# 3dlg-hcvc/tricolo

Measured on AMD Instinct MI355X. Metric: trimodal training samples/sec (32^3 voxel + 6-view), higher is better.
Workload: dtype f16 (f16 activation storage + f16 MFMA operands, fp32 accumulate; bf16x3 heads/GRU; within 1e-3 of the fp32 reference)

## Files before the change

### include/tricolo_hip.h

```cpp
#ifndef TRICOLO_HIP_H
#define TRICOLO_HIP_H
#include <stddef.h>
#include <stdint.h>

#ifdef __cplusplus
extern "C" {
#endif

#define TRI_FMT_F32 0
#define TRI_FMT_BF16 1
#define TRI_FMT_F16 2

int tri_version(void);
const char* tri_last_error(void);

typedef struct TriConvDesc {
    int B, ID, IH, IW, Cin;
    int OD, OH, OW, Cout;
    int KD, KH, KW, stride, pad_d, pad_h, pad_w;
} TriConvDesc;

int tri_conv_kpad(int ntaps, int cin_stored);
typedef struct TriPrepDesc {
    const float* w;
// ... 24 lines not shown

int tri_conv_num_mtiles(const TriConvDesc* d, int split3);
int tri_conv_num_records(const TriConvDesc* d, int split3, int row_list);
int tri_conv_kernel_family(const TriConvDesc* d, int transposed, int split3);
int tri_conv_wgrad_kernel_family(const TriConvDesc* d, int act_fmt);
size_t tri_conv_workspace(const TriConvDesc* d, int transposed);
int tri_conv_fwd(const TriConvDesc* d, const void* in, const void* w_hi, const void* w_lo, void* out, const uint8_t* row_mask,
                 const float* bias, int act, int accumulate, float* stats, int act_fmt, void* workspace, size_t workspace_bytes,
                 const int* row_pos , const int* row_count ,
                 void* stream);
int tri_conv_dgrad(const TriConvDesc* d, const void* dout, const void* wt_hi, const void* wt_lo, void* din, const uint8_t* row_mask,
                   int accumulate, int act_fmt, void* workspace, size_t workspace_bytes,
                   const int* row_pos ,
                   const int* row_count ,
                   void* stream);
typedef struct TriConvBnSums {
    const void* y;
    const float* relu_scale;
    const float* relu_shift;
    const void* relu_out;
    float* partial;
} TriConvBnSums;
int tri_conv_dgrad_bn_records(const TriConvDesc* d, int accumulate, int act_fmt);
int tri_conv_dgrad_bn(const TriConvDesc* d, const void* dout, const void* wt_hi, const void* wt_lo, void* din, int accumulate,
                      int act_fmt, void* workspace, size_t workspace_bytes, const int* row_pos, const TriConvBnSums* sums, void* stream);
size_t tri_conv_wgrad_workspace(const TriConvDesc* d);
size_t tri_conv_plan_bytes(const TriConvDesc* d);
int tri_conv_plan_build(const TriConvDesc* d, void* plan, void* stream);
int tri_conv_wgrad(const TriConvDesc* d, const void* in, const void* dout, const uint8_t* row_mask, const void* plan ,
                   void* workspace, size_t workspace_bytes, float* dw, long s_co, long s_tap, long s_ci, int cin_real, int split3,
                   int act_fmt, float out_scale ,
                   const int* row_pos, const int* row_count ,
                   void* stream);
#ifndef TRI_WGRAD_GROUP_MAX
#define TRI_WGRAD_GROUP_MAX 24
#endif
typedef struct TriWgradReduce {
    const float* slab;
    float* dw;
    long s_co, s_tap, s_ci;
    int splits, Cout, Kpad, ntaps, cin_stored, cin_real, zlanes, nblocks;
    float out_scale;
    int kw_real;
    int kw_shift;
} TriWgradReduce;
int tri_conv_wgrad_partial(const TriConvDesc* d, const void* in, const void* dout, const uint8_t* row_mask, const void* plan ,
// ... 154 lines not shown
```

### tricolo_amd/_C.py

```python
from __future__ import annotations

import ctypes as C
import os

import torch

_HERE = os.path.dirname(os.path.abspath(__file__))
LIB_PATH = os.path.join(_HERE, "libtricolo_hip.so")


class TriConvDesc(C.Structure):
    _fields_ = [(n, C.c_int) for n in ("B", "ID", "IH", "IW", "Cin", "OD", "OH", "OW", "Cout",
                                       "KD", "KH", "KW", "stride", "pad_d", "pad_h", "pad_w")]


class TriPrepDesc(C.Structure):
    _fields_ = [("w", C.c_void_p), ("hi", C.c_void_p), ("lo", C.c_void_p), ("s_row", C.c_long), ("s_tap", C.c_long),
                ("s_inner", C.c_long), ("rows", C.c_int), ("ntaps", C.c_int), ("inner", C.c_int), ("inner_pad", C.c_int),
                ("kpad", C.c_int), ("fmt", C.c_int), ("frag", C.c_int)]


class TriWgradReduce(C.Structure):
    _fields_ = [("slab", C.c_void_p), ("dw", C.c_void_p), ("s_co", C.c_long), ("s_tap", C.c_long), ("s_ci", C.c_long)] + \
               [(n, C.c_int) for n in ("splits", "Cout", "Kpad", "ntaps", "cin_stored", "cin_real", "zlanes", "nblocks")] + \
# ... 18 lines not shown

SIGNATURES = {
    "tri_version": (I, []),
    "tri_last_error": (C.c_char_p, []),
    "tri_conv_kpad": (I, [I, I]),
    "tri_weight_prep": (I, [P, L, L, L, I, I, I, I, P, P, I, I, P]),
    "tri_weight_prep_multi": (I, [P, I, P]),
    "tri_embedding_fwd": (I, [P, P, I, I, I, P, P]),
    "tri_embedding_bwd": (I, [P, P, I, I, I, I, I, P, P]),
    "tri_retrieval_topk": (I, [P, P, P, I, I, I, I, P, P, P, P]),
    "tri_linear_small_supported": (I, [I, I, I]),
    "tri_linear_small_fwd": (I, [P, P, P, P, I, I, I, I, I, P]),
    "tri_linear_small_dgrad": (I, [P, P, P, P, I, I, I, I, I, P]),
    "tri_linear_small_wgrad": (I, [P, P, P, P, P, I, I, I, I, I, P]),
    "tri_linear_small_bwd": (I, [P, P, P, P, P, P, P, I, I, I, I, I, P]),
    "tri_conv_num_mtiles": (I, [DP, I]),
    "tri_conv_num_records": (I, [DP, I, I]),
    "tri_conv_workspace": (Z, [DP, I]),
    "tri_conv_kernel_family": (I, [DP, I, I]),
    "tri_conv_wgrad_kernel_family": (I, [DP, I]),
    "tri_conv_fwd": (I, [DP, P, P, P, P, P, P, I, I, P, I, P, Z, P, P, P]),
    "tri_conv_dgrad": (I, [DP, P, P, P, P, P, I, I, P, Z, P, P, P]),
    "tri_conv_dgrad_bn_records": (I, [DP, I, I]),
    "tri_conv_dgrad_bn": (I, [DP, P, P, P, P, I, I, P, Z, P, C.POINTER(TriConvBnSums), P]),
    "tri_conv_wgrad_workspace": (Z, [DP]),
    "tri_conv_plan_bytes": (Z, [DP]),
    "tri_conv_plan_build": (I, [DP, P, P]),
    "tri_conv_wgrad": (I, [DP, P, P, P, P, P, Z, P, L, L, L, I, I, I, F, P, P, P]),
    "tri_conv_wgrad_partial": (I, [DP, P, P, P, P, P, Z, P, L, L, L, I, I, I, F, P, P, P, P]),
    "tri_wgrad_reduce_grouped": (I, [P, I, P]),
    "tri_wgrad_reduce_grouped_noted": (I, [P, I, P, P]),
    "tri_conv_stem_wgrad_bn": (I, [DP, P, P, P, P, P, P, P, P, P, P, Z, P, L, L, L, I, I, F, P, P]),
    "tri_conv_wgrad_group_info": (I, [DP, I, P, P, P]),
    "tri_conv_wgrad_partial_group": (I, [P, I, I, P, P]),
    "tri_bn_finalize": (I, [P, I, I, P, I, P, P, P, P, P, F, F, P, P, P, P, P]),
    "tri_bn_eval_coeffs": (I, [I, P, P, P, P, F, P, P, P, P, P]),
    "tri_bn_act": (I, [P, P, P, P, P, P, P, L, I, I, I, P]),
    "tri_relu_bwd": (I, [P, P, P, L, I, P]),
    "tri_bn_bwd_num_blocks": (I, [L]),
    "tri_bn_bwd_reduce": (I, [P, P, L, I, P, P, P, P, P, I, P]),
    "tri_bn_bwd_finalize": (I, [P, I, I, P, I, P, P, P, P, P, P, P, P, F, P]),
    "tri_bn_bwd_small": (I, [P, P, L, I, P, I, P, P, P, P, P, P, P, P, I, P, P, P, F, I, P]),
    "tri_bn_bwd_apply": (I, [P, P, P, P, P, P, P, L, I, P, P, P, P, I, I, P]),
    "tri_bn_bwd_pair_reduce": (I, [P, P, P, P, L, I, P, P, I, P]),
    "tri_bn_bwd_pair_finalize": (I, [P, P, I, I, I, P, P, P, P, P, P, P, P, F, P]),
    "tri_bn_bwd_pair_apply": (I, [P, P, P, P, P, P, P, P, P, L, I, I, P]),
# ... 130 lines not shown
```

### tricolo_amd/csrc/conv_igemm.hip

```cpp
#include "common.h"
#include <stdlib.h>
#include <map>
#include <mutex>
#include "../../include/tricolo_hip.h"
#include "conv_vox.h"

struct ConvArgs {
    const void* in;
    const void* w_hi;
    const void* w_lo;
    void* out;
    const uint8_t* row_mask;
    const int* row_pos;
    const int* row_count;
    const float* bias;
    float* stats;
    float* slab;
    int B, ID, IH, IW, Cin;
    int OD, OH, OW, Cout;
    int KD, KH, KW, stride, pd, ph, pw;
    int transposed, act, accumulate;
    int Kpad, M, ntaps, cin_shift, ksplit, steps_per_split;
    unsigned in_bytes;
    int nunits;
    int h_tr, h_rows, h_slab_bytes, h_nr, h_mtiles;
    int h_dbuf;
    int h_abl;
    int h_xcg, h_touch;
    int h_swz;
#ifdef HALO_STAMPS
    long long* h_dbg;
#endif
    FastDiv dOW, dOH, dOD, dCin, dP, dH2;
};

template <int N>
__device__ __forceinline__ float row_ror(float v) {
    return __builtin_bit_cast(float, __builtin_amdgcn_update_dpp(0, __builtin_bit_cast(int, v), 0x120 + N, 0xf, 0xf, false));
}

template <typename AT, int BN, int TM, int TN, int WAVES_M, int WM, int WN>
__device__ __forceinline__ void conv_epilogue(const ConvArgs& p, f32x4 (&acc)[TM][TN], int m0, int n0, int mtile, int wm, int wn, int fr,
                                              int fq, int t, int split, int any_active, float* red, int Meff) {
    if (p.ksplit > 1) {
        if (!any_active) return;
        float* slab = p.slab + (size_t)split * p.M * p.Cout;
#pragma unroll
        for (int a = 0; a < TM; ++a) {
            int m = m0 + wm * WM + a * 16 + fr;
            if (m < Meff)
#pragma unroll
                for (int b = 0; b < TN; ++b) {
                    int n = n0 + wn * WN + b * 16 + fq * 4;
                    *(f32x4*)(slab + (size_t)m * p.Cout + n) = acc[a][b];
                }
        }
// ... 544 lines not shown
        stats[((size_t)rec * 2 + 1) * Cout + ntile * BN + t] = q_;
    }
}

__device__ __forceinline__ v4i lds_read16(unsigned addr) {
    v4i r;
    asm volatile("ds_read_b128 %0, %1" : "=v"(r) : "v"(addr));
    return r;
}
template <int OFF>
__device__ __forceinline__ v4i lds_read16_off(unsigned addr) {
    v4i r;
    asm volatile("ds_read_b128 %0, %1 offset:%2" : "=v"(r) : "v"(addr), "n"(OFF));
    return r;
}
template <int N>
__device__ __forceinline__ void frag_wait(v4i (&a)[2], v4i (&b)[4]) {
    asm volatile("s_waitcnt lgkmcnt(%6)" : "+v"(a[0]), "+v"(a[1]), "+v"(b[0]), "+v"(b[1]), "+v"(b[2]), "+v"(b[3]) : "n"(N));
}
template <int N>
__device__ __forceinline__ void frag_wait(v4i (&a)[3], v4i (&b)[4]) {
    asm volatile("s_waitcnt lgkmcnt(%7)" : "+v"(a[0]), "+v"(a[1]), "+v"(a[2]), "+v"(b[0]), "+v"(b[1]), "+v"(b[2]), "+v"(b[3]) : "n"(N));
}
#ifdef HALO_STAMPS
#define HSTAMP(id) do { if (wave == 0 && n_stamp < 255) { const long long c_ = __builtin_readcyclecounter(); if (lane == 0) stl[n_stamp] = ((long long)(id) << 48) | (c_ & 0xFFFFFFFFFFFFll); ++n_stamp; } } while (0)
#else
#define HSTAMP(id) do { } while (0)
#endif
template <int TM, bool WGREC, typename AT>
__global__ __launch_bounds__(256, WGREC ? 3 : 1) void conv_halo2d_kernel(const ConvArgs p) {
    typedef Mma<typename OpOf<AT>::E> MM;
    typedef typename MM::v8 v8;
    constexpr int BN = 64, TN = 4, WM = 16 * TM, W_BYTES = BN * 128, NR = HALO_NR;
    extern __shared__ __attribute__((aligned(16))) char smem[];
    const int slab_bytes = p.h_slab_bytes;
    char* const ring = smem + slab_bytes;
    float* const red = (float*)(ring + NR * W_BYTES);

    const int t = threadIdx.x, lane = t & 63, wave = t >> 6;
    const int fr = lane & 15, fq = lane >> 4;
#ifdef HALO_STAMPS
    int n_stamp = 0;
    long long* const stl = (long long*)(smem + p.h_slab_bytes + HALO_NR * 8192 + 2048);
#endif
    HSTAMP(1);
    const int H = p.IH, W = p.IW, P = W + 2, TR = p.h_tr, NH = p.B * H;
    const int NT = p.Cout / BN, nchunks = p.Cin >> 6;
    const int items = p.h_mtiles * NT, G = gridDim.x;
    const int S = slab_bytes >> 12;
    const int zero_pix = p.h_rows * P;
    const v4i in_rsrc = make_rsrc_words(p.in, p.in_bytes);
    const v4i w_rsrc = make_rsrc_words(p.w_hi, (unsigned)((size_t)p.Cout * p.Kpad * 2));
    const unsigned lds_slab = lds_addr(smem) + wave * 1024, lds_ring = lds_addr(ring) + wave * 1024;
// ... 76 lines not shown
        }
    };

    int item = blockIdx.x;
    if (item >= items) return;
    HSTAMP(2);
    {
        issue_slab((item / NT) * TR, 0);
#pragma unroll
        for (int d = 0; d < NR - 1; ++d) issue_w();
    }
    int c_slot = 0;
    f32x4 cs[TN], cq[TN];
#pragma unroll
    for (int b = 0; b < TN; ++b) { cs[b] = (f32x4){0.f, 0.f, 0.f, 0.f}; cq[b] = cs[b]; }
    for (; item < items; item += G) {
        const int mtile = item / NT, ntile = item - mtile * NT;
        if (!WGREC) {
#pragma unroll
            for (int b = 0; b < TN; ++b) { cs[b] = (f32x4){0.f, 0.f, 0.f, 0.f}; cq[b] = cs[b]; }
        }
        const int g0 = mtile * TR;
        const int npos = min(TR, NH - g0) * W;
        int pix0[TM], tmul[TM];
#pragma unroll
        for (int a = 0; a < TM; ++a) {
            const bool ok = wave * WM + a * 16 + fr < npos;
            pix0[a] = ok ? pixc[a] : zero_pix;
            tmul[a] = ok ? 1 : 0;
        }
        f32x4 acc[TM][TN];
#pragma unroll
        for (int a = 0; a < TM; ++a)
#pragma unroll
            for (int b = 0; b < TN; ++b) acc[a][b] = (f32x4){0.f, 0.f, 0.f, 0.f};

        for (int chunk = 0; chunk < nchunks; ++chunk) {
            if (chunk > 0) {
                __builtin_amdgcn_s_barrier();
                asm volatile("" ::: "memory");
                issue_slab(g0, chunk);
            }
            HSTAMP(3);
            asm volatile("s_waitcnt vmcnt(0)" ::: "memory");
            HSTAMP(4);
            int shift = p.transposed ? (P + 1) : -(P + 1), kx = 0;
            int gshift = p.transposed ? (p.h_swz + 1) : -(p.h_swz + 1);
#pragma unroll 1
            for (int tap = 0; tap < 9; ++tap) {
                --w_ahead;
                if (tap > 0 && !(p.h_abl & 64)) {
                    if (w_ahead == NR - 2) wait_vmcnt_c<2 * (NR - 2)>();
                    else wait_vmcnt(2 * w_ahead);
                }
                HSTAMP(5);
                __builtin_amdgcn_s_barrier();
                asm volatile("" ::: "memory");
                HSTAMP(6);
// ... 14 lines not shown
                        for (int a = 0; a < TM; ++a) ar[kk][a] = lds_read16(aaddr[a] ^ (kk << 6));
#pragma unroll
                        for (int b = 0; b < TN; ++b) br[kk][b] = lds_read16_off<0>(wb + boff[kk] + b * 2048);
                    }
                    frag_wait<TM + TN>(ar[0], br[0]);
#pragma unroll
                    for (int b = 0; b < TN; ++b)
#pragma unroll
                        for (int a = 0; a < TM; ++a) acc[a][b] = MM::mma(__builtin_bit_cast(v8, br[0][b]), __builtin_bit_cast(v8, ar[0][a]), acc[a][b]);
                    frag_wait<0>(ar[1], br[1]);
#pragma unroll
                    for (int b = 0; b < TN; ++b)
#pragma unroll
                        for (int a = 0; a < TM; ++a) acc[a][b] = MM::mma(__builtin_bit_cast(v8, br[1][b]), __builtin_bit_cast(v8, ar[1][a]), acc[a][b]);
                }
                HSTAMP(8);
                if (++c_slot == NR) c_slot = 0;
                const int step = (++kx == 3) ? (kx = 0, P - 2) : 1;
                const int gstep = kx == 0 ? p.h_swz - 2 : 1;
                shift += p.transposed ? -step : step;
                gshift += p.transposed ? -gstep : gstep;
            }
        }
        __builtin_amdgcn_s_barrier();
        asm volatile("" ::: "memory");
        if (item + G < items) issue_slab(((item + G) / NT) * TR, 0);

        HSTAMP(9);
        if (!(p.h_abl & 4)) {
            AT* const out = (AT*)p.out + ((size_t)g0 * W) * p.Cout + ntile * BN;
#pragma unroll
            for (int a = 0; a < TM; ++a) {
                const int m = wave * WM + a * 16 + fr;
                if (m < npos) {
#pragma unroll
                    for (int b = 0; b < TN; ++b) {
                        AT* o = out + (size_t)m * p.Cout + b * 16 + fq * 4;
                        f32x4 v = acc[a][b];
                        if (p.accumulate) { float4 e = Act<AT>::ld4(o); v[0] += e.x; v[1] += e.y; v[2] += e.z; v[3] += e.w; }
                        Act<AT>::st4(o, make_float4(v[0], v[1], v[2], v[3]));
                        if (p.stats) {
                            v[0] = Act<AT>::rnd(v[0]); v[1] = Act<AT>::rnd(v[1]); v[2] = Act<AT>::rnd(v[2]); v[3] = Act<AT>::rnd(v[3]);
                            cs[b] += v;
                            cq[b] += v * v;
                        }
                    }
                }
            }
            HSTAMP(10);
            if (!WGREC && p.stats && !(p.h_abl & 16)) halo_store_stats<TN, BN>(cs, cq, red, p.stats, p.Cout, mtile, ntile, wave, fr, fq, t, true);
        }
        HSTAMP(11);
    }
#ifdef HALO_STAMPS
    if (wave == 0) {
        asm volatile("s_waitcnt lgkmcnt(0)" ::: "memory");
        for (int i = lane; i < 255; i += 64) p.h_dbg[(size_t)blockIdx.x * 256 + i] = i < n_stamp ? stl[i] : 0;
        if (lane == 0) p.h_dbg[(size_t)blockIdx.x * 256 + 255] = n_stamp;
    }
#endif
    if (WGREC && p.stats && !(p.h_abl & 16)) halo_store_stats<TN, BN>(cs, cq, red, p.stats, p.Cout, blockIdx.x / NT, blockIdx.x % NT, wave, fr, fq, t, false);
}


// ... 1180 lines not shown
                for (int tap = 0; tap < 9; ++tap)
                    for (int kk = 0; kk < 2; ++kk)
                        for (int g = 0; g < 4; ++g) {
                            int cnt[16] = {0}, mx = 0;
                            for (int l = 0; l < 16; ++l) {
                                const int lane = grp[g][l], fr = lane & 15, fq = lane >> 4;
                                const int pa = wave * 16 * TM + a * 16 + fr, j = pa / W, x = pa - j * W, i = whole ? j / H : 0;
                                const int row = j + 1 + 2 * i + tap / 3 - 1, col = x + 1 + tap % 3 - 1;
                                const int slot = (((row * P + col) & 1) << 3) | (((fq + 4 * kk) ^ (col + c1 * row)) & 7);
                                if (++cnt[slot] > mx) mx = cnt[slot];
                            }
                            cyc += mx;
                        }
        if (best < 0 || cyc < best) { best = cyc; best_c = c1; }
    }
    std::lock_guard<std::mutex> lk(mu);
    memo[key] = best_c;
    return best_c;
}

#ifdef HALO_STAMPS
static long long* g_halo_dbg = nullptr;
#endif
template <int TM, typename AT>
static int launch_halo(ConvArgs& a, const ConvPlan& pl, hipStream_t stream) {
    a.h_tr = pl.h_tr; a.h_rows = pl.h_rows; a.h_slab_bytes = pl.h_slab_bytes; a.h_nr = pl.h_nr; a.h_mtiles = pl.h_mtiles;
    a.h_dbuf = pl.h_dbuf;
    a.h_abl = tri_probe_ablation();
    a.dP = make_fastdiv(a.IW + 2); a.dH2 = make_fastdiv(a.IH + 2);
    a.h_swz = halo_swizzle(a.IW, a.IH, pl.halo);
#ifdef HALO_STAMPS
    a.h_dbg = g_halo_dbg;
    const size_t smem = (size_t)pl.h_slab_bytes + (size_t)HALO_NR * 8192 + 2048 + 2048;
#else
    const size_t smem = (size_t)pl.h_slab_bytes + (size_t)HALO_NR * 8192 + 2048;
#endif
    a.h_xcg = 0; a.h_touch = 0;
    if (pl.h_v5) {
        static int xcg_on = -1, touch_on = -1;
        if (xcg_on < 0) { const char* e = getenv("TRICOLO_HALO_XCG"); xcg_on = e ? atoi(e) : -1; if (xcg_on < 0) xcg_on = 99; }
        if (touch_on < 0) { const char* e = getenv("TRICOLO_HALO_TOUCH"); touch_on = (e && e[0] == '0') ? 0 : 1; }
        const int NT = a.Cout / 64, G = pl.h_grid;
        if (xcg_on && G == pl.h_mtiles * NT && G % 8 == 0 && a.Cin != 64) {
            const double wb = (double)a.Cout * a.Kpad * 2, ib = (double)a.M * a.Cin * 2;
            double best = 0;
            for (int cg = 1; cg <= NT; ++cg) {
                if (NT % cg || 8 % (NT / cg) || (G / 8) % cg) continue;
                if (xcg_on != 99 && cg != xcg_on) continue;
// ... 14 lines not shown
#ifdef HALO_NTL_EXPERIMENT
        { static int f = -1; if (f < 0) f = 0;
          const int items = pl.h_mtiles * (a.Cout / 64), per_wg = (items + pl.h_grid - 1) / pl.h_grid;
          if (f && a.Cin != 64 && per_wg > 1) ntl = per_wg == 2 ? 2 : 4; }
#endif
#define TRI_ROWS_LAUNCH(DRIP_, ACC_, NTL_, ...)                                                                                     \
        do {                                                                                                                        \
            static size_t attr5 = 0;                                                                                                \
            if (smem5 > attr5) {                                                                                                    \
                hipFuncSetAttribute((const void*)conv_halo_rows_kernel<AT, DRIP_, ACC_, NTL_, ##__VA_ARGS__>, hipFuncAttributeMaxDynamicSharedMemorySize, \
                                    (int)smem5);                                                                                    \
                attr5 = smem5;                                                                                                      \
            }                                                                                                                       \
            conv_halo_rows_kernel<AT, DRIP_, ACC_, NTL_, ##__VA_ARGS__><<<pl.h_grid, 256, smem5, stream>>>(a);                       \
        } while (0)
#define TRI_ROWS_MODE(NTL_)                                                                                                         \
        do {                                                                                                                        \
            if (a.accumulate) TRI_ROWS_LAUNCH(false, true, NTL_);                                                                   \
            else if (drip) TRI_ROWS_LAUNCH(true, false, NTL_);                                                                      \
            else TRI_ROWS_LAUNCH(false, false, NTL_);                                                                               \
        } while (0)
        static int prod = -1;
        if (prod < 0) { const char* e = getenv("TRICOLO_HALO_PROD"); prod = (e && e[0] == '0') ? 0 : 1; }
        if (prod && pl.halo == 2 && ntl == 0) {
#define TRI_ROWS_LAUNCH_P(DRIP_, ACC_)                                                                                              \
        do {                                                                                                                        \
            static size_t attrp = 0;                                                                                                \
            if (smem5 > attrp) {                                                                                                    \
                hipFuncSetAttribute((const void*)conv_halo_rows_kernel<AT, DRIP_, ACC_, 0, 2, true>, hipFuncAttributeMaxDynamicSharedMemorySize, \
                                    (int)smem5);                                                                                    \
                attrp = smem5;                                                                                                      \
            }                                                                                                                       \
            conv_halo_rows_kernel<AT, DRIP_, ACC_, 0, 2, true><<<pl.h_grid, 512, smem5, stream>>>(a);                                \
        } while (0)
            if (a.accumulate) TRI_ROWS_LAUNCH_P(false, true);
            else if (drip) TRI_ROWS_LAUNCH_P(true, false);
            else TRI_ROWS_LAUNCH_P(false, false);
#undef TRI_ROWS_LAUNCH_P
            return tri_check_launch("tri_conv(halo rows, producer waves)");
        }
        if (pl.halo == 3) {
            if (a.accumulate) TRI_ROWS_LAUNCH(false, true, 0, 3);
            else TRI_ROWS_LAUNCH(false, false, 0, 3);
        }
        else if (ntl == 0) TRI_ROWS_MODE(0);
        else if (ntl == 1) TRI_ROWS_MODE(1);
#ifdef HALO_NTL_EXPERIMENT
        else if (ntl == 2) TRI_ROWS_MODE(2);
        else TRI_ROWS_MODE(4);
#endif
#undef TRI_ROWS_MODE
#undef TRI_ROWS_LAUNCH
        return tri_check_launch("tri_conv(halo rows)");
    }
    static size_t attr = 0;
    if (smem > attr) {
        hipFuncSetAttribute((const void*)conv_halo2d_kernel<TM, false, AT>, hipFuncAttributeMaxDynamicSharedMemorySize, (int)smem);
        hipFuncSetAttribute((const void*)conv_halo2d_kernel<TM, true, AT>, hipFuncAttributeMaxDynamicSharedMemorySize, (int)smem);
        attr = smem;
    }
    if (pl.h_wgrec && a.stats) conv_halo2d_kernel<TM, true, AT><<<pl.h_grid, 256, smem, stream>>>(a);
    else conv_halo2d_kernel<TM, false, AT><<<pl.h_grid, 256, smem, stream>>>(a);
    return tri_check_launch("tri_conv(halo)");
}

template <typename AT>
static int launch_stem(ConvArgs& a, hipStream_t stream) {
    StemGeom sg;
    a.h_abl = tri_probe_ablation();
    if (!stem_geometry(a.B, a.IH, a.IW, a.Cin, a.OH, a.OW, a.Cout, a.KD, a.KH, a.KW, a.stride, a.pd, a.ph, a.pw, &sg)) {
        tri_set_error("conv(stem): geometry changed between plan and launch"); return TRI_ERR_ARG;
    }
    const size_t smem = (size_t)2 * sg.slab_rows * sg.row_bytes + 4 * 64 * 2 * sizeof(float);
#define TRI_STEM(KH_)                                                                                                     \
    case KH_: {                                                                                                           \
        static bool attr = false;                                                                                         \
        if (!attr) {                                                                                                      \
            hipFuncSetAttribute((const void*)conv_stem_kernel<KH_, 2, AT>, hipFuncAttributeMaxDynamicSharedMemorySize, 80 * 1024); \
            hipFuncSetAttribute((const void*)conv_stem_kernel<KH_, 4, AT>, hipFuncAttributeMaxDynamicSharedMemorySize, 80 * 1024); \
            attr = true;                                                                                                  \
        }                                                                                                                 \
        if (sg.npt == 4) conv_stem_kernel<KH_, 4, AT><<<sg.grid, 256, smem, stream>>>(a, sg);                             \
// ... 94 lines not shown
            return tri_internal_c64_launch(cg, a.B, a.IH, a.in, a.w_hi, a.out, bs ? bs->partial : a.stats, a.transposed, a.accumulate, act_fmt, bs, stream);
        }
        if (a.stats) {
            tri_set_error("conv: this layer runs conv_c64_kernel (tri_conv_kernel_family == 9): statistics only without row mask / bias / activation");
            return TRI_ERR_ARG;
        }
        a.row_pos = a.row_count ? a.row_pos : nullptr;
    }
    if (pl.s2g) {
        if (a.transposed || a.row_mask || a.row_count || a.bias || a.act != 0 || a.accumulate) {
            tri_set_error("conv: this layer runs conv_s2g_kernel (tri_conv_kernel_family == 15): forward only, no row mask / list, bias, activation "
                          "or accumulate");
            return TRI_ERR_ARG;
        }
        TriS2gGeom g2;
        tri_internal_s2g_geometry(a.B, a.ID, a.IH, a.IW, a.Cin, a.OD, a.OH, a.OW, a.Cout, a.KD, a.KH, a.KW, a.stride, a.pd, a.ph, a.pw, &g2);
        return tri_internal_s2g_launch(g2, a.B, a.IH, a.IW, a.Cin, a.Cout, a.Kpad, a.in, a.w_hi, a.out, a.stats, act_fmt, stream);
    }
    if (pl.s2d && a.transposed && !bs && !a.row_mask && !a.row_count && !a.bias && a.act == 0 && !a.stats) {
        TriC64Geom sg;
        tri_internal_s2d_geometry(a.B, a.ID, a.IH, a.IW, a.Cin, a.OD, a.OH, a.OW, a.Cout, a.KD, a.KH, a.KW, a.stride, a.pd, a.ph, a.pw, &sg);
        return tri_internal_s2d_launch(sg, a.B, a.IH, a.in, a.w_hi, a.out, a.accumulate, act_fmt, stream);
    }
    if (bs) {
        tri_set_error("conv: this layer's data-gradient kernel takes no BatchNorm-backward sums (tri_conv_dgrad_bn_records == 0)");
        return TRI_ERR_UNSUPPORTED;
    }
    if (pl.stem && !a.transposed && !a.row_mask && !a.row_count && !a.bias && a.act == 0 && !a.accumulate) {
        a.row_pos = nullptr;
        return act_fmt == TRI_FMT_F16 ? launch_stem<f16_t>(a, stream) : launch_stem<bf16_t>(a, stream);
    }
    if (pl.halo && !a.row_mask && !a.row_count && !a.bias && a.act == 0) {
        a.row_pos = nullptr;
        return act_fmt == TRI_FMT_F16 ? launch_halo<2, f16_t>(a, pl, stream) : launch_halo<2, bf16_t>(a, pl, stream);
    }
    if (pl.pw && pl.pw_tr == (a.transposed ? 1 : 0) && !a.row_mask && !a.row_count && !a.bias && a.act == 0 && !a.accumulate) {
        TriPwGeom pg;
        tri_internal_pw_geometry(a.B, a.ID, a.IH, a.IW, a.Cin, a.OD, a.OH, a.OW, a.Cout, a.KD, a.KH, a.KW, a.stride, a.pd, a.ph, a.pw, &pg);
        return tri_internal_pw_launch(pg, a.B, a.in, a.w_hi, a.Cin, a.Cout, a.Kpad, a.out, a.stats, a.transposed ? 1 : 0, act_fmt, stream);
    }
    if (pl.dma) return act_fmt == TRI_FMT_F16 ? launch_dma_any<f16_t>(a, pl.bn, stream) : launch_dma_any<bf16_t>(a, pl.bn, stream);
#define TRI_CONV(BN_)                                                                                     \
    (act_fmt == TRI_FMT_F16 ? launch_conv<BN_, 1, f16_t>(a, stream)                                       \
     : act_fmt == TRI_FMT_BF16 ? launch_conv<BN_, 1, bf16_t>(a, stream)                                   \
     : (split ? launch_conv<BN_, 2, float>(a, stream) : launch_conv<BN_, 1, float>(a, stream)))
    if (a.Cout % 128 == 0 && pl.bn != 64) return TRI_CONV(128);
    if (a.Cout % 64 == 0) return TRI_CONV(64);
    return TRI_CONV(32);
#undef TRI_CONV
}

extern "C" int tri_conv_kpad(int ntaps, int cin_stored) { return (ntaps * cin_stored + 31) / 32 * 32; }

extern "C" int tri_conv_num_records(const TriConvDesc* d, int split3, int row_list) {
    long M = (long)d->B * d->OD * d->OH * d->OW;
    ConvPlan pl = conv_make_plan(d->B, d->ID, d->IH, d->IW, d->Cin, d->OD, d->OH, d->OW, d->Cout, d->KD, d->KH, d->KW, d->stride, d->pad_d,
                                 d->pad_h, d->pad_w, split3, row_list);
// ... 66 lines not shown
extern "C" int tri_conv_dgrad(const TriConvDesc* d, const void* dout, const void* wt_hi, const void* wt_lo, void* din,
                              const uint8_t* row_mask, int accumulate, int act_fmt, void* workspace, size_t workspace_bytes,
                              const int* row_pos, const int* row_count, void* stream) {
    ConvArgs a{};
    a.in = dout; a.w_hi = wt_hi; a.w_lo = wt_lo; a.out = din;
    a.row_mask = row_mask; a.bias = nullptr; a.stats = nullptr; a.row_pos = row_pos; a.row_count = row_count;
    a.B = d->B; a.ID = d->OD; a.IH = d->OH; a.IW = d->OW; a.Cin = d->Cout;
    a.OD = d->ID; a.OH = d->IH; a.OW = d->IW; a.Cout = d->Cin;
    a.KD = d->KD; a.KH = d->KH; a.KW = d->KW; a.stride = d->stride; a.pd = d->pad_d; a.ph = d->pad_h; a.pw = d->pad_w;
    a.transposed = 1; a.act = 0; a.accumulate = accumulate;
    a.ntaps = d->KD * d->KH * d->KW;
    a.M = d->B * d->ID * d->IH * d->IW;
    return conv_dispatch(a, act_fmt, workspace, workspace_bytes, (hipStream_t)stream);
}

extern "C" int tri_conv_dgrad_bn_records(const TriConvDesc* d, int accumulate, int act_fmt) {
    (void)accumulate;
    if (act_fmt != TRI_FMT_BF16 && act_fmt != TRI_FMT_F16) return 0;
    ConvPlan pl = conv_make_plan(d->B, d->OD, d->OH, d->OW, d->Cout, d->ID, d->IH, d->IW, d->Cin, d->KD, d->KH, d->KW, d->stride, d->pad_d,
                                 d->pad_h, d->pad_w, 2, 0);
    if (pl.c64 && d->IW <= 32) return pl.c64_grid;
    return 0;
}
extern "C" int tri_conv_dgrad_bn(const TriConvDesc* d, const void* dout, const void* wt_hi, const void* wt_lo, void* din, int accumulate,
                                 int act_fmt, void* workspace, size_t workspace_bytes, const int* row_pos, const TriConvBnSums* sums,
                                 void* stream) {
    if (!sums || !sums->y || !sums->partial || (!sums->relu_scale != !sums->relu_shift) || (sums->relu_scale && sums->relu_out)) {
        tri_set_error("tri_conv_dgrad_bn: sums needs y, partial and at most one of (relu_scale + relu_shift) / relu_out");
        return TRI_ERR_ARG;
    }
    if (tri_conv_dgrad_bn_records(d, accumulate, act_fmt) == 0) {
        tri_set_error("tri_conv_dgrad_bn: no fused form for this layer (tri_conv_dgrad_bn_records == 0)");
        return TRI_ERR_UNSUPPORTED;
    }
    ConvArgs a{};
    a.in = dout; a.w_hi = wt_hi; a.w_lo = wt_lo; a.out = din;
    a.row_pos = row_pos;
    a.B = d->B; a.ID = d->OD; a.IH = d->OH; a.IW = d->OW; a.Cin = d->Cout;
    a.OD = d->ID; a.OH = d->IH; a.OW = d->IW; a.Cout = d->Cin;
    a.KD = d->KD; a.KH = d->KH; a.KW = d->KW; a.stride = d->stride; a.pd = d->pad_d; a.ph = d->pad_h; a.pw = d->pad_w;
    a.transposed = 1; a.act = 0; a.accumulate = accumulate;
    a.ntaps = d->KD * d->KH * d->KW;
    a.M = d->B * d->ID * d->IH * d->IW;
    return conv_dispatch(a, act_fmt, workspace, workspace_bytes, (hipStream_t)stream, sums);
}
```

### tricolo_amd/model/module/img_encoder/mv_cnn.py

```python
from __future__ import annotations

import os

import torch
import torch.nn as nn

from .... import ops
from ....layers import SideStream, TriModule, linear_bwd, linear_fwd, require_gpu


_DS_FWD = int(os.environ.get("TRICOLO_DS_FWD", "2"))
_DS_BWD = int(os.environ.get("TRICOLO_DS_BWD", "2"))
_PREP_DGRAD_LATE = os.environ.get("TRICOLO_PREP_DGRAD_LATE", "1") != "0"
_BN_PAIR = True
_STEM_BESIDE_WGRAD = os.environ.get("TRICOLO_STEM_BESIDE_WGRAD", "1") != "0"
_PREP_ISSUE = int(os.environ.get("TRICOLO_PREP_ISSUE", "1"))


class _BasicBlockParams(nn.Module):
    def __init__(self, inplanes, planes, stride):
        super().__init__()
        self.conv1 = nn.Conv2d(inplanes, planes, 3, stride, 1, bias=False)
        self.bn1 = nn.BatchNorm2d(planes)
        self.relu = nn.ReLU(inplace=True)
# ... 279 lines not shown
            g = dout
            fine = ops.TIMELINE is not None and ops.TIMELINE.get("fine")
            tag = f"image.bwd.c{y2.shape[-1]}.b{bi}"
            if fine:
                ops.stamp(tag + ".bn2")
            mode = _DS_BWD if (blk.downsample is not None and batch is not None) else 0
            ev = None
            if mode == 2:
                ev = torch.cuda.Event()
                ev.record()

            def shortcut_bwd():
                with torch.cuda.stream(self._side_ds.fork(g, yd, event=ev)):
                    if dyd_pair is not None:
                        return dyd_pair, ops.conv_dgrad(dyd_pair, gd, self._packed[(id(blk.downsample[0]), True)])
                    dyd_, gr[blk.downsample[1].weight], gr[blk.downsample[1].bias] = ops.bn_bwd(
                        yd, g, cod, blk.downsample[1].weight, count_host=gd.M, inplace=False, out_scale=ugs)
                    if batch is None:
                        gr[blk.downsample[0].weight] = ops.conv_wgrad(x, dyd_, gd, blk.downsample[0].weight, prec, out_scale=ugs)
                    return dyd_, ops.conv_dgrad(dyd_, gd, self._packed[(id(blk.downsample[0]), True)])
            if blk.downsample is not None and not mode:
                dyd, dx = shortcut_bwd()
            wgrad_async(a1, dy2, g2, blk.conv2.weight)
            da1, sums1 = ops.conv_dgrad(dy2, g2, self._packed[(id(blk.conv2), True)], bn_sums=(y1, co1, None))
            if mode:
                dyd, dx = shortcut_bwd()
            if fine:
                ops.stamp(tag + ".dgrad2")
            dy1, gr[blk.bn1.weight], gr[blk.bn1.bias] = ops.bn_bwd(y1, da1, co1, blk.bn1.weight, count_host=g1.M, relu=True, out_scale=ugs,
                                                                   partial=sums1)
            if fine:
                ops.stamp(tag + ".bn1")
            wgrad_async(x, dy1, g1, blk.conv1.weight)
            if blk.downsample is not None:
                if batch is None:
                    self._side_ds.join(dx, gr[blk.downsample[0].weight], gr[blk.downsample[1].weight], gr[blk.downsample[1].bias])
                else:
                    self._side_ds.join(dx, dyd, gr[blk.downsample[1].weight], gr[blk.downsample[1].bias])
                    gr[blk.downsample[0].weight] = ops.conv_wgrad(x, dyd, gd, blk.downsample[0].weight, prec, out_scale=ugs, batch=batch)
            else:
                dx = g
            if bi > 0:
                prev = saved_blocks[bi - 1]
                dx, dout_sums = ops.conv_dgrad(dy1, g1, self._packed[(id(blk.conv1), True)], out=dx, accumulate=True,
                                               bn_sums=(prev[5], None, prev[11]))
            else:
                dx, dout_sums = ops.conv_dgrad(dy1, g1, self._packed[(id(blk.conv1), True)], out=dx, accumulate=True), None
# ... 134 lines not shown
```

### tricolo_amd/ops.py

```python
from __future__ import annotations

import math
import os

import torch

from . import _C
from ._C import check, lib, make_desc, ptr, stream

_PRECISIONS = ("bf16", "bf16x3", "f16")
_FMT = {torch.float32: 0, torch.bfloat16: 1, torch.float16: 2}
F16_GRAD_SCALE = float(os.environ.get("TRICOLO_F16_GRAD_SCALE", "4096"))
if not (F16_GRAD_SCALE >= 1.0 and math.frexp(F16_GRAD_SCALE)[0] == 0.5):
    raise ValueError(f"TRICOLO_F16_GRAD_SCALE={F16_GRAD_SCALE!r}: must be a power of two >= 1 (the kernels divide it out exactly)")
_default_precision = os.environ.get("TRICOLO_PRECISION", "bf16x3")


def set_default_precision(p: str):
    global _default_precision
    if p not in _PRECISIONS:
        raise ValueError(f"precision must be one of {_PRECISIONS}")
    _default_precision = p


# ... 198 lines not shown
        return t

    def brick(self, transposed: bool, mode: int) -> bool:
        return (self.kernel_family[(transposed, mode)] & 255) in (6, 7, 13, 14)

    def packed_frag(self, transposed: bool, precision: str, storage=None) -> int:
        storage = storage or act_dtype(precision)
        mode = 1 if precision == "bf16x3" else (2 if storage != torch.float32 else 0)
        return 1 if (self.kernel_family[(transposed, mode)] & 255) in _FRAG_FAMILIES else 0

    def check_packed(self, packed, transposed: bool, x):
        need = 1 if (self.kernel_family[(transposed, _conv_mode(x, packed[1]))] & 255) in _FRAG_FAMILIES else 0
        if getattr(packed[0], "tri_frag", 0) != need:
            raise RuntimeError("conv: the packed operand was ordered for another plan (row-major vs fragment-major): pack it with "
                               "pack_weight(..., storage=<dtype of the activations>)")

    def voxg_spu(self, transposed: bool, mode: int) -> int:
        code = self.kernel_family[(transposed, mode)]
        return (code >> 24) & 127 if (code & 255) == 13 else 0

    def splitk(self, transposed: bool, mode: int) -> bool:
        return bool(self.kernel_family[(transposed, mode)] >> 16 & 1)

    def dgrad_bn_records(self, accumulate: bool, fmt: int) -> int:
        c = self.__dict__.setdefault("_dgrad_bn", {})
        k = (bool(accumulate), fmt)
        if k not in c:
            c[k] = int(lib().tri_conv_dgrad_bn_records(_C.C.byref(self.desc), 1 if accumulate else 0, fmt))
        return c[k]

    def wgrad_group(self, fmt: int):
        c = self.__dict__.setdefault("_wgrad_group", {})
        if fmt not in c:
            fam, tiles, steps = _C.C.c_int(), _C.C.c_int(), _C.C.c_int()
            check(lib().tri_conv_wgrad_group_info(_C.C.byref(self.desc), fmt, _C.C.byref(fam), _C.C.byref(tiles), _C.C.byref(steps)),
                  "tri_conv_wgrad_group_info")
            c[fmt] = (fam.value, tiles.value, steps.value)
        return c[fmt]

    def plan(self, device):
        pl = self._plans.get(device)
        if pl is None:
            pl = torch.empty((lib().tri_conv_plan_bytes(_C.C.byref(self.desc)),), dtype=torch.uint8, device=device)
            check(lib().tri_conv_plan_build(_C.C.byref(self.desc), ptr(pl), stream()), "tri_conv_plan_build")
            self._plans[device] = pl
        return pl

    @property
    def flops(self):
        return 2 * self.M * self.ntaps * self.cin * self.cout

# ... 63 lines not shown
    g.check_packed(packed, False, x)
    OD, OH, OW = g.out_grid
    if out is None:
        out = torch.empty((g.B, OD, OH, OW, g.cout), dtype=x.dtype, device=x.device)
    assert out.dtype == x.dtype
    nrec = (g.num_records_rows if rows else g.num_mtiles)[_conv_mode(x, lo)]
    stats = torch.empty((nrec, 2, g.cout), dtype=torch.float32, device=x.device) if want_stats else None
    ws = _workspace(g.fwd_ws, x.device) if g.fwd_ws else None
    check(_timed(_igemm_symbol(g, False, lo is not None, x), _flops(g, rows, row_mask),
                 lambda: lib().tri_conv_fwd(_C.C.byref(g.desc), ptr(_act(x)), ptr(hi), ptr(lo), ptr(out), ptr(row_mask), ptr(bias),
                                            act, 1 if accumulate else 0, ptr(stats), _abf(x), ptr(ws),
                                            ws.numel() if ws is not None else 0, ptr(rows[0]) if rows else None,
                                            ptr(rows[1]) if rows else None, stream())), "tri_conv_fwd")
    return (out, stats) if want_stats else out


_ROW_ORDER = True


_DGRAD_BN_MODE = os.environ.get("TRICOLO_DGRAD_BN", "2")
_DGRAD_BN = _DGRAD_BN_MODE != "0"


def conv_dgrad(dout, g: ConvGeom, packed_t, row_mask=None, out=None, accumulate=False, rows=None, bn_sums=None):
    hi, lo = packed_t
    g.check_packed(packed_t, True, dout)
    ID, IH, IW = g.in_grid
    if out is None:
        out = torch.empty((g.B, ID, IH, IW, g.cin_stored), dtype=dout.dtype, device=dout.device)
    assert out.dtype == dout.dtype
    ws = _workspace(g.dgrad_ws, dout.device) if g.dgrad_ws else None
    rowpos = g.dgrad_row_order(dout.device) if (row_mask is None and rows is None and _ROW_ORDER) else None
    if rows is not None:
        rowpos = rows[0]
    if bn_sums is not None:
        y, co, relu_out = bn_sums
        nrec = g.dgrad_bn_records(accumulate, _abf(dout)) if (_DGRAD_BN and not (accumulate and _DGRAD_BN_MODE == "2") and row_mask is None and rows is None and lo is None
                                                               and (relu_out is not None) == bool(accumulate)
                                                               and (co is not None) != (relu_out is not None)) else 0
        if nrec == 0:
            return conv_dgrad(dout, g, packed_t, row_mask=row_mask, out=out, accumulate=accumulate, rows=rows), None
        assert y.dtype == out.dtype and y.numel() == out.numel()
        partial = torch.empty((nrec, 2, g.cin_stored), dtype=torch.float32, device=dout.device)
        sums = _C.TriConvBnSums(ptr(y), ptr(co.scale) if co is not None else None, ptr(co.shift) if co is not None else None,
                                ptr(relu_out), ptr(partial))
        check(_timed(_igemm_symbol(g, True, False, dout), g.flops,
                     lambda: lib().tri_conv_dgrad_bn(_C.C.byref(g.desc), ptr(_act(dout)), ptr(hi), None, ptr(out), 1 if accumulate else 0,
                                                     _abf(dout), ptr(ws), ws.numel() if ws is not None else 0, ptr(rowpos),
                                                     _C.C.byref(sums), stream())), "tri_conv_dgrad_bn")
        return out, partial
    check(_timed(_igemm_symbol(g, True, lo is not None, dout), _flops(g, rows, row_mask),
                 lambda: lib().tri_conv_dgrad(_C.C.byref(g.desc), ptr(_act(dout)), ptr(hi), ptr(lo), ptr(out), ptr(row_mask),
                                              1 if accumulate else 0, _abf(dout), ptr(ws), ws.numel() if ws is not None else 0,
                                              ptr(rowpos), ptr(rows[1]) if rows else None, stream())), "tri_conv_dgrad")
    return out


_wgrad_ws = {}


# ... 861 lines not shown
```

Before: 13350.

## Fuse BatchNorm-backward sums into halo conv dgrad kernel for MV-CNN blocks

Adds a SUMS variant of the halo 2D conv kernel that, during the data-gradient epilogue, loads the forward activation y plus the BN scale/shift, applies the ReLU mask and accumulates per-channel sum and sum-of-products partials. A new records_ex query enables this fused path for transposed, non-accumulating halo layers, and the multi-view CNN conv2 backward opts into it. This removes a separate BN-backward reduction pass over the gradient and activation tensors. In exchange it adds extra loads and registers to the epilogue, with a launch-bounds change to occupancy 3 that may constrain registers.

```diff
diff --git a/include/tricolo_hip.h b/include/tricolo_hip.h
--- a/include/tricolo_hip.h
+++ b/include/tricolo_hip.h
@@ -70,6 +70,7 @@
     float* partial;
 } TriConvBnSums;
 int tri_conv_dgrad_bn_records(const TriConvDesc* d, int accumulate, int act_fmt);
+int tri_conv_dgrad_bn_records_ex(const TriConvDesc* d, int accumulate, int act_fmt);
 int tri_conv_dgrad_bn(const TriConvDesc* d, const void* dout, const void* wt_hi, const void* wt_lo, void* din, int accumulate,
                       int act_fmt, void* workspace, size_t workspace_bytes, const int* row_pos, const TriConvBnSums* sums, void* stream);
 size_t tri_conv_wgrad_workspace(const TriConvDesc* d);
diff --git a/tricolo_amd/_C.py b/tricolo_amd/_C.py
--- a/tricolo_amd/_C.py
+++ b/tricolo_amd/_C.py
@@ -64,6 +64,7 @@
     "tri_conv_fwd": (I, [DP, P, P, P, P, P, P, I, I, P, I, P, Z, P, P, P]),
     "tri_conv_dgrad": (I, [DP, P, P, P, P, P, I, I, P, Z, P, P, P]),
     "tri_conv_dgrad_bn_records": (I, [DP, I, I]),
+    "tri_conv_dgrad_bn_records_ex": (I, [DP, I, I]),
     "tri_conv_dgrad_bn": (I, [DP, P, P, P, P, I, I, P, Z, P, C.POINTER(TriConvBnSums), P]),
     "tri_conv_wgrad_workspace": (Z, [DP]),
     "tri_conv_plan_bytes": (Z, [DP]),
diff --git a/tricolo_amd/csrc/conv_igemm.hip b/tricolo_amd/csrc/conv_igemm.hip
--- a/tricolo_amd/csrc/conv_igemm.hip
+++ b/tricolo_amd/csrc/conv_igemm.hip
@@ -32,6 +32,9 @@
     long long* h_dbg;
 #endif
     FastDiv dOW, dOH, dOD, dCin, dP, dH2;
+    const void* bs_y;
+    const float* bs_scale;
+    const float* bs_shift;
 };
 
 template <int N>
@@ -622,13 +625,23 @@
 __device__ __forceinline__ void frag_wait(v4i (&a)[3], v4i (&b)[4]) {
     asm volatile("s_waitcnt lgkmcnt(%7)" : "+v"(a[0]), "+v"(a[1]), "+v"(a[2]), "+v"(b[0]), "+v"(b[1]), "+v"(b[2]), "+v"(b[3]) : "n"(N));
 }
+template <typename AT>
+__device__ __forceinline__ void halo_bn_sums(f32x4 v, uint2 y4, const f32x4& sc, const f32x4& sh, f32x4& cs, f32x4& cq) {
+    typedef AT at4 __attribute__((ext_vector_type(4)));
+    const at4 yh = __builtin_bit_cast(at4, y4);
+    const f32x4 yf = {(float)yh[0], (float)yh[1], (float)yh[2], (float)yh[3]};
+#pragma unroll
+    for (int r = 0; r < 4; ++r) v[r] = __fmaf_rn(yf[r], sc[r], sh[r]) > 0.f ? v[r] : 0.f;
+    cs += v;
+    cq += v * yf;
+}
 #ifdef HALO_STAMPS
 #define HSTAMP(id) do { if (wave == 0 && n_stamp < 255) { const long long c_ = __builtin_readcyclecounter(); if (lane == 0) stl[n_stamp] = ((long long)(id) << 48) | (c_ & 0xFFFFFFFFFFFFll); ++n_stamp; } } while (0)
 #else
 #define HSTAMP(id) do { } while (0)
 #endif
-template <int TM, bool WGREC, typename AT>
-__global__ __launch_bounds__(256, WGREC ? 3 : 1) void conv_halo2d_kernel(const ConvArgs p) {
+template <int TM, bool WGREC, typename AT, bool SUMS = false>
+__global__ __launch_bounds__(256, (WGREC || SUMS) ? 3 : 1) void conv_halo2d_kernel(const ConvArgs p) {
     typedef Mma<typename OpOf<AT>::E> MM;
     typedef typename MM::v8 v8;
     constexpr int BN = 64, TN = 4, WM = 16 * TM, W_BYTES = BN * 128, NR = HALO_NR;
@@ -751,6 +764,10 @@
         }
         const int g0 = mtile * TR;
         const int npos = min(TR, NH - g0) * W;
+        unsigned warm = 0;
+        if constexpr (SUMS) {
+            if (t < npos) warm = *(const unsigned*)((const AT*)p.bs_y + ((size_t)g0 * W + t) * p.Cout + ntile * BN);
+        }
         int pix0[TM], tmul[TM];
 #pragma unroll
         for (int a = 0; a < TM; ++a) {
@@ -763,6 +780,7 @@
         for (int a = 0; a < TM; ++a)
 #pragma unroll
             for (int b = 0; b < TN; ++b) acc[a][b] = (f32x4){0.f, 0.f, 0.f, 0.f};
+        if constexpr (SUMS) asm volatile("" :: "v"(warm));
 
         for (int chunk = 0; chunk < nchunks; ++chunk) {
             if (chunk > 0) {
@@ -823,6 +841,22 @@
                 gshift += p.transposed ? -gstep : gstep;
             }
         }
+        uint2 ybs[TM][TN];
+        f32x4 bsc[TN], bsh[TN];
+        if constexpr (SUMS) {
+            const AT* const yt = (const AT*)p.bs_y + ((size_t)g0 * W) * p.Cout + ntile * BN + fq * 4;
+#pragma unroll
+            for (int a = 0; a < TM; ++a) {
+                const int m = wave * WM + a * 16 + fr;
+#pragma unroll
+                for (int b = 0; b < TN; ++b) ybs[a][b] = m < npos ? *(const uint2*)(yt + (size_t)m * p.Cout + b * 16) : make_uint2(0u, 0u);
+            }
+#pragma unroll
+            for (int b = 0; b < TN; ++b) {
+                bsc[b] = *(const f32x4*)(p.bs_scale + ntile * BN + b * 16 + fq * 4);
+                bsh[b] = *(const f32x4*)(p.bs_shift + ntile * BN + b * 16 + fq * 4);
+            }
+        }
         __builtin_amdgcn_s_barrier();
         asm volatile("" ::: "memory");
         if (item + G < items) issue_slab(((item + G) / NT) * TR, 0);
@@ -840,7 +874,10 @@
                         f32x4 v = acc[a][b];
                         if (p.accumulate) { float4 e = Act<AT>::ld4(o); v[0] += e.x; v[1] += e.y; v[2] += e.z; v[3] += e.w; }
                         Act<AT>::st4(o, make_float4(v[0], v[1], v[2], v[3]));
-                        if (p.stats) {
+                        if constexpr (SUMS) {
+                            v[0] = Act<AT>::rnd(v[0]); v[1] = Act<AT>::rnd(v[1]); v[2] = Act<AT>::rnd(v[2]); v[3] = Act<AT>::rnd(v[3]);
+                            halo_bn_sums<AT>(v, ybs[a][b], bsc[b], bsh[b], cs[b], cq[b]);
+                        } else if (p.stats) {
                             v[0] = Act<AT>::rnd(v[0]); v[1] = Act<AT>::rnd(v[1]); v[2] = Act<AT>::rnd(v[2]); v[3] = Act<AT>::rnd(v[3]);
                             cs[b] += v;
                             cq[b] += v * v;
@@ -2067,8 +2104,14 @@
 #ifdef HALO_STAMPS
 static long long* g_halo_dbg = nullptr;
 #endif
+static int halo_dgrad_bn_records(const ConvPlan& pl, int cout, long M, int accumulate) {
+    if (!pl.halo || pl.h_v5 || pl.h_wgrec || pl.h_grid != pl.h_mtiles * (cout / 64) || accumulate || M * cout * 2 >= ((long)1 << 31)) return 0;
+    return pl.h_mtiles;
+}
+
 template <int TM, typename AT>
-static int launch_halo(ConvArgs& a, const ConvPlan& pl, hipStream_t stream) {
+static int launch_halo(ConvArgs& a, const ConvPlan& pl, hipStream_t stream, const TriConvBnSums* bs = nullptr) {
+    if (bs) { a.stats = bs->partial; a.bs_y = bs->y; a.bs_scale = bs->relu_scale; a.bs_shift = bs->relu_shift; }
     a.h_tr = pl.h_tr; a.h_rows = pl.h_rows; a.h_slab_bytes = pl.h_slab_bytes; a.h_nr = pl.h_nr; a.h_mtiles = pl.h_mtiles;
     a.h_dbuf = pl.h_dbuf;
     a.h_abl = tri_probe_ablation();
@@ -2129,6 +2172,10 @@
         } while (0)
         static int prod = -1;
         if (prod < 0) { const char* e = getenv("TRICOLO_HALO_PROD"); prod = (e && e[0] == '0') ? 0 : 1; }
+        if (bs) {
+            tri_set_error("conv(halo rows): no BatchNorm-backward sums form (tri_conv_dgrad_bn_records_ex == 0)");
+            return TRI_ERR_UNSUPPORTED;
+        }
         if (prod && pl.halo == 2 && ntl == 0) {
 #define TRI_ROWS_LAUNCH_P(DRIP_, ACC_)                                                                                              \
         do {                                                                                                                        \
@@ -2165,6 +2212,19 @@
         hipFuncSetAttribute((const void*)conv_halo2d_kernel<TM, false, AT>, hipFuncAttributeMaxDynamicSharedMemorySize, (int)smem);
         hipFuncSetAttribute((const void*)conv_halo2d_kernel<TM, true, AT>, hipFuncAttributeMaxDynamicSharedMemorySize, (int)smem);
         attr = smem;
+    }
+    if (bs) {
+        if (a.accumulate || pl.h_wgrec) {
+            tri_set_error("conv(halo): no BatchNorm-backward sums form for this launch (tri_conv_dgrad_bn_records_ex == 0)");
+            return TRI_ERR_UNSUPPORTED;
+        }
+        static size_t attrs = 0;
+        if (smem > attrs) {
+            hipFuncSetAttribute((const void*)conv_halo2d_kernel<TM, false, AT, true>, hipFuncAttributeMaxDynamicSharedMemorySize, (int)smem);
+            attrs = smem;
+        }
+        conv_halo2d_kernel<TM, false, AT, true><<<pl.h_grid, 256, smem, stream>>>(a);
+        return tri_check_launch("tri_conv(halo, BatchNorm-backward sums)");
     }
     if (pl.h_wgrec && a.stats) conv_halo2d_kernel<TM, true, AT><<<pl.h_grid, 256, smem, stream>>>(a);
     else conv_halo2d_kernel<TM, false, AT><<<pl.h_grid, 256, smem, stream>>>(a);
@@ -2305,8 +2365,8 @@
         tri_internal_s2d_geometry(a.B, a.ID, a.IH, a.IW, a.Cin, a.OD, a.OH, a.OW, a.Cout, a.KD, a.KH, a.KW, a.stride, a.pd, a.ph, a.pw, &sg);
         return tri_internal_s2d_launch(sg, a.B, a.IH, a.in, a.w_hi, a.out, a.accumulate, act_fmt, stream);
     }
-    if (bs) {
-        tri_set_error("conv: this layer's data-gradient kernel takes no BatchNorm-backward sums (tri_conv_dgrad_bn_records == 0)");
+    if (bs && !(a.transposed && bs->relu_scale && halo_dgrad_bn_records(pl, a.Cout, a.M, a.accumulate))) {
+        tri_set_error("conv: this layer's data-gradient kernel takes no BatchNorm-backward sums (tri_conv_dgrad_bn_records[_ex] == 0)");
         return TRI_ERR_UNSUPPORTED;
     }
     if (pl.stem && !a.transposed && !a.row_mask && !a.row_count && !a.bias && a.act == 0 && !a.accumulate) {
@@ -2315,7 +2375,7 @@
     }
     if (pl.halo && !a.row_mask && !a.row_count && !a.bias && a.act == 0) {
         a.row_pos = nullptr;
-        return act_fmt == TRI_FMT_F16 ? launch_halo<2, f16_t>(a, pl, stream) : launch_halo<2, bf16_t>(a, pl, stream);
+        return act_fmt == TRI_FMT_F16 ? launch_halo<2, f16_t>(a, pl, stream, bs) : launch_halo<2, bf16_t>(a, pl, stream, bs);
     }
     if (pl.pw && pl.pw_tr == (a.transposed ? 1 : 0) && !a.row_mask && !a.row_count && !a.bias && a.act == 0 && !a.accumulate) {
         TriPwGeom pg;
@@ -2428,6 +2488,13 @@
     if (pl.c64 && d->IW <= 32) return pl.c64_grid;
     return 0;
 }
+extern "C" int tri_conv_dgrad_bn_records_ex(const TriConvDesc* d, int accumulate, int act_fmt) {
+    const int n = tri_conv_dgrad_bn_records(d, accumulate, act_fmt);
+    if (n || (act_fmt != TRI_FMT_BF16 && act_fmt != TRI_FMT_F16)) return n;
+    ConvPlan pl = conv_make_plan(d->B, d->OD, d->OH, d->OW, d->Cout, d->ID, d->IH, d->IW, d->Cin, d->KD, d->KH, d->KW, d->stride, d->pad_d,
+                                 d->pad_h, d->pad_w, 2, 0);
+    return halo_dgrad_bn_records(pl, d->Cin, (long)d->B * d->ID * d->IH * d->IW, accumulate);
+}
 extern "C" int tri_conv_dgrad_bn(const TriConvDesc* d, const void* dout, const void* wt_hi, const void* wt_lo, void* din, int accumulate,
                                  int act_fmt, void* workspace, size_t workspace_bytes, const int* row_pos, const TriConvBnSums* sums,
                                  void* stream) {
@@ -2435,8 +2502,8 @@
         tri_set_error("tri_conv_dgrad_bn: sums needs y, partial and at most one of (relu_scale + relu_shift) / relu_out");
         return TRI_ERR_ARG;
     }
-    if (tri_conv_dgrad_bn_records(d, accumulate, act_fmt) == 0) {
-        tri_set_error("tri_conv_dgrad_bn: no fused form for this layer (tri_conv_dgrad_bn_records == 0)");
+    if (tri_conv_dgrad_bn_records_ex(d, accumulate, act_fmt) == 0) {
+        tri_set_error("tri_conv_dgrad_bn: no fused form for this layer (tri_conv_dgrad_bn_records_ex == 0)");
         return TRI_ERR_UNSUPPORTED;
     }
     ConvArgs a{};
diff --git a/tricolo_amd/model/module/img_encoder/mv_cnn.py b/tricolo_amd/model/module/img_encoder/mv_cnn.py
--- a/tricolo_amd/model/module/img_encoder/mv_cnn.py
+++ b/tricolo_amd/model/module/img_encoder/mv_cnn.py
@@ -325,7 +325,7 @@
             if blk.downsample is not None and not mode:
                 dyd, dx = shortcut_bwd()
             wgrad_async(a1, dy2, g2, blk.conv2.weight)
-            da1, sums1 = ops.conv_dgrad(dy2, g2, self._packed[(id(blk.conv2), True)], bn_sums=(y1, co1, None))
+            da1, sums1 = ops.conv_dgrad(dy2, g2, self._packed[(id(blk.conv2), True)], bn_sums=(y1, co1, None), bn_sums_ex=True)
             if mode:
                 dyd, dx = shortcut_bwd()
             if fine:
diff --git a/tricolo_amd/ops.py b/tricolo_amd/ops.py
--- a/tricolo_amd/ops.py
+++ b/tricolo_amd/ops.py
@@ -244,11 +244,12 @@
     def splitk(self, transposed: bool, mode: int) -> bool:
         return bool(self.kernel_family[(transposed, mode)] >> 16 & 1)
 
-    def dgrad_bn_records(self, accumulate: bool, fmt: int) -> int:
+    def dgrad_bn_records(self, accumulate: bool, fmt: int, ex: bool = False) -> int:
         c = self.__dict__.setdefault("_dgrad_bn", {})
-        k = (bool(accumulate), fmt)
+        k = (bool(accumulate), fmt, bool(ex))
         if k not in c:
-            c[k] = int(lib().tri_conv_dgrad_bn_records(_C.C.byref(self.desc), 1 if accumulate else 0, fmt))
+            query = lib().tri_conv_dgrad_bn_records_ex if ex else lib().tri_conv_dgrad_bn_records
+            c[k] = int(query(_C.C.byref(self.desc), 1 if accumulate else 0, fmt))
         return c[k]
 
     def wgrad_group(self, fmt: int):
@@ -358,7 +359,7 @@
 _DGRAD_BN = _DGRAD_BN_MODE != "0"
 
 
-def conv_dgrad(dout, g: ConvGeom, packed_t, row_mask=None, out=None, accumulate=False, rows=None, bn_sums=None):
+def conv_dgrad(dout, g: ConvGeom, packed_t, row_mask=None, out=None, accumulate=False, rows=None, bn_sums=None, bn_sums_ex=False):
     hi, lo = packed_t
     g.check_packed(packed_t, True, dout)
     ID, IH, IW = g.in_grid
@@ -371,7 +372,7 @@
         rowpos = rows[0]
     if bn_sums is not None:
         y, co, relu_out = bn_sums
-        nrec = g.dgrad_bn_records(accumulate, _abf(dout)) if (_DGRAD_BN and not (accumulate and _DGRAD_BN_MODE == "2") and row_mask is None and rows is None and lo is None
+        nrec = g.dgrad_bn_records(accumulate, _abf(dout), bn_sums_ex) if (_DGRAD_BN and not (accumulate and _DGRAD_BN_MODE == "2") and row_mask is None and rows is None and lo is None
                                                                and (relu_out is not None) == bool(accumulate)
                                                                and (co is not None) != (relu_out is not None)) else 0
         if nrec == 0:
```

Result: no change. 13350 (median of 2 runs) (+0.1%).
